# meco-group/omg-tools

Hardware: AMD Instinct MI355X
Metric: MPC solves/sec, 1024-agent Holonomic Point2point batch per GPU (higher is better)
Workload: dtype f64

## Files before the change

### omg-tools_amd/csrc/omgx.hip

```cpp
#include <hip/hip_runtime.h>
#include <hip/hip_ext.h>
#include <stdarg.h>
#include <stdio.h>
#include <stdlib.h>
#include <string.h>
#include <string>
#include <vector>
#include "../../include/omgx.h"
#include "omgx_core.h"
#include "omgx_plan.h"
#include "omgx_kernels.h"
#include "omgx_table_cache.h"

namespace {

thread_local std::string g_err;

#define HIPCHK(call)                                                              \
  do {                                                                            \
    hipError_t e_ = (call);                                                       \
    if (e_ != hipSuccess) {                                                       \
      g_err = std::string(#call) + ": " + hipGetErrorString(e_);                  \
      return OMGX_E_HIP;                                                          \
    }                                                                             \
// ... 343 lines not shown
        if (ad >= 0) { b->ev_hess.push_back(ad); b->ev_hess.push_back(plan.order[q1]); b->ev_hess.push_back(plan.order[q2]); }
      }
  }
  UP(prog, 6 * d.n_prog); UP(knots, t->n_knots); UP(pp_ptr, t->n_pp + 1); UP(pm_coef, t->n_mono);
  UP(pm_ptr, t->n_mono + 1); UP(pm_atom, t->n_matom); UP(slot_pp, d.n_slots);
  if (d.mono_packed == 2) {
    TRY(upload(img, plan.pm_rec8.data(), plan.pm_rec8.size(), (const omgx::MonoRec8**)&b->dev.pm_rec));
    TRY(upload(img, plan.sl_ell8.data(), plan.sl_ell8.size(), (const omgx::MonoRec8**)&b->dev.sl_ell));
  } else { UP(pm_rec, plan.pm_rec.size()); UP(sl_ell, plan.sl_ell.size()); }
  UP(row_ptr, d.n_con + 2); UP(t_coef, d.n_terms); UP(t_slot, d.n_terms); UP(t_var, OMGX_TERM_VARS * d.n_terms);
  UP(order, d.N); UP(leaf_off, d.n_leaf + 1); UP(leaf_bw, plan.leaf_bw.size()); UP(blk, d.N);
  UP(eq_rows, d.n_eq); UP(eq_index, d.n_con);
  UP(cpl_ptr, d.n_leaf + 1); UP(cpl_idx, plan.cpl_idx.size()); UP(cpl_map, plan.cpl_map.size());
  UP(d_off, d.n_leaf + 1); UP(b_off, plan.b_off.size());
  UP(lf_w, plan.lf_w.size()); UP(lf_ldb, plan.lf_ldb.size()); UP(lf_band, plan.lf_band.size()); UP(lf_kind, plan.lf_kind.size()); UP(dl_pos, plan.dl_pos.size());
  UP(pair4, plan.pair4.size()); UP(eqe3, plan.eqe3.size());
  UP(je_row, plan.je_row.size()); UP(diag_addr, d.N); UP(tq_addr, plan.tq_addr.size());
  UP(reg_w, d.N); UP(je_rp, plan.je_rp.size());
  UP(slot_rng, plan.slot_rng.size());
  UP(row_perm, plan.row_perm.size()); UP(cs_ptr, plan.cs_ptr.size()); UP(cs_rec, plan.cs_rec.size());
  UP(obj_ent, plan.obj_ent.size());
  UP(ka_rec, plan.ka_rec.size()); UP(kh_rec, plan.kh_rec.size()); UP(kg_rec, plan.kg_rec.size());
  UP(ka_fix, plan.ka_fix.size()); UP(kg_fix, plan.kg_fix.size()); UP(kh_fix, plan.kh_fix.size());
  UP(rt_ell, plan.rt_ell.size()); UP(rt_glen, plan.rt_glen.size()); UP(jp_ell, plan.jp_ell.size()); UP(jp_glen, plan.jp_glen.size());
  UP(cs_ell, plan.cs_ell.size()); UP(cs_glen, plan.cs_glen.size()); UP(cs_col, plan.cs_col.size()); UP(cs_own, plan.cs_own.size());
  UP(jv_ell, plan.jv_ell.size()); UP(jv_own, plan.jv_own.size()); UP(jv_glen, plan.jv_glen.size());
  UP(ja_ell, plan.ja_ell.size()); UP(ja_own, plan.ja_own.size()); UP(ja_glen, plan.ja_glen.size());
  UP(sl_list, plan.sl_list.size()); UP(sl_glen, plan.sl_glen.size());
  UP(lift_rec, plan.lift_rec.size()); UP(lift_lev, plan.lift_lev.size());
  return bind_tables(b, img);
// ... 432 lines not shown
    hipExtLaunchKernelGGL(b->inst.prepare, dim3(B), dim3(b->threads), (uint32_t)b->prep_lds, b->stream, e0, nullptr, 0u, d, b->dev, b->opts,
                          kp, kx0, klb, kub, shared ? 1 : 0, (const double*)klam, (const int32_t*)kst, B, b->d_prep, b->prep_doubles, (flags & OMGX_ONLY_FAILED) ? 1 : 0);
    HIPCHK(hipGetLastError());
    e0 = nullptr;
  }
  const StoreArgs* k_stp = (b->store.out || b->signals.log) ? &b->d_store->st : nullptr;
  const int k_only_failed = (flags & OMGX_ONLY_FAILED) ? 1 : 0, k_n_alt = b->d_x0_alt ? b->n_alt : 0;
  const CenterArgs* k_ctr = b->center_on ? b->d_center : nullptr;
  double* k_prep = prepared ? b->d_prep : nullptr;
  const StopArgs* k_stop = b->stop_on ? b->d_stop : nullptr;
  const bool lean_launch = !k_stp && !k_only_failed && !k_n_alt && !b->d_attempts && !k_ctr && !k_prep && !k_stop &&
                           !(b->opts.compl_tol > 0.0) && !(b->opts.viol_tol > 0.0) && !b->opts.refine;
  const Instances& in = b->inst;
  b->last_instance = lean_launch && in.lean ? 1 : 0;
  const ipm_kernel_t kern = b->last_instance ? in.lean : (b->opts.refine && in.refine ? in.refine : in.full);
  hipExtLaunchKernelGGL(kern, dim3(b->n_slabs), dim3(b->threads), (uint32_t)b->lds_bytes, b->stream,
                        e0, e1, 0u, d, b->dev,
                        b->opts, b->kkt_doubles, kp, kx0, klb, kub, shared ? 1 : 0, kx, klam, kst, kit, B, b->d_prof,
                        b->d_slabs, b->slab_doubles, b->d_dw, b->d_order, k_stp, k_only_failed,
                        b->d_next, b->d_x0_alt, k_n_alt, b->d_attempts,
                        (unsigned long long*)(b->d_stats ? b->d_stats + 4 * (size_t)(b->stats_launch++ % b->stats_slots) : nullptr),
                        b->stagger, k_ctr, k_prep, b->prep_doubles, k_stop);
  HIPCHK(hipGetLastError());
  if (ranged)
    hipLaunchKernelGGL(range_contract_lam, dim3((B * nu + 255) / 256), dim3(256), 0, b->stream, (const double*)b->d_lam, lam_user_dev, B, nu, ni,
                       (const int32_t*)b->d_range_dup);
  if (!dev) {
    HIPCHK(hipMemcpyAsync(x, b->d_x, (size_t)B * d.n_var * sizeof(double), hipMemcpyDeviceToHost, b->stream));
    HIPCHK(hipMemcpyAsync(lam_g, ranged ? b->d_lam_user : b->d_lam, (size_t)B * nu * sizeof(double), hipMemcpyDeviceToHost, b->stream));
    HIPCHK(hipMemcpyAsync(status, b->d_status, (size_t)B * sizeof(int32_t), hipMemcpyDeviceToHost, b->stream));
    HIPCHK(hipMemcpyAsync(iters, b->d_iters, (size_t)B * sizeof(int32_t), hipMemcpyDeviceToHost, b->stream));
    HIPCHK(hipStreamSynchronize(b->stream));
  }
  return OMGX_OK;
}
// ... 535 lines not shown
  }
  a.iters_log = sp->iters_log; a.status_log = sp->status_log;
  a.plant = b->plant_on ? b->d_plant : nullptr;
  a.script = b->script_on ? b->d_script : nullptr;
  const ipm_rollout_t kern = b->script_on ? (b->plant_on ? b->inst.rollout_plant_script : b->inst.rollout_script)
                                          : (b->plant_on ? b->inst.rollout_plant : b->inst.rollout);
  HIPCHK(hipMemcpyAsync(b->ro_steps.p, steps.data(), sizeof(RolloutStep) * steps.size(), hipMemcpyHostToDevice, b->stream));
  TRY(push_args(b, &b->d_rollout, a));
  TRY(flush_order(b));
  const bool shared = flags & OMGX_BOUNDS_SHARED;
  hipEvent_t e0 = b->ext_ev0, e1 = b->ext_ev0 ? b->ext_ev1 : nullptr;
  b->ext_ev0 = b->ext_ev1 = nullptr;
  b->timed = false;
  hipExtLaunchKernelGGL(kern, dim3(b->n_slabs < b->n_agents ? b->n_slabs : b->n_agents), dim3(b->threads), (uint32_t)b->lds_bytes, b->stream, e0, e1, 0u,
                        d, b->dev, b->opts, b->kkt_doubles, p, x, lbg, ubg, shared ? 1 : 0, lam_g, status, iters, b->n_agents,
                        b->d_slabs, b->slab_doubles, b->d_dw, b->d_next, (const RolloutArgs*)b->d_rollout, b->stagger, b->d_order,
                        (const StoreArgs*)((b->store.out || b->signals.log) ? &b->d_store->st : nullptr));
  HIPCHK(hipGetLastError());
  return OMGX_OK;
}

int omgx_batch_predict_ex(omgx_batch* b, const double* x, double* p, int32_t coeff_off, int32_t n_spl, int32_t degree,
                          const double* knots, int32_t n_knots, double tau, double inv_T, int32_t n_out,
                          const int32_t* p_off, int32_t p_t, double t_value, int32_t mode, const double* state_in,
                          int32_t n_sub, double dtau) {
  const Plan pl{coeff_off, n_spl, degree, n_knots, inv_T, knots};
  TRY(check_predict("predict", pl, 1, kAnySpl, x, p, p_off, n_out));
  if (mode != OMGX_PREDICT_IDEAL && mode != OMGX_PREDICT_RK4) return bad("predict: mode = %d is neither OMGX_PREDICT_IDEAL nor OMGX_PREDICT_RK4", mode);
  if (mode == OMGX_PREDICT_RK4 && (!state_in || n_sub < 1 || !(dtau > 0.0) || n_out < 2))
    return bad("predict: OMGX_PREDICT_RK4 needs state_in, n_sub >= 1, dtau > 0 and n_out >= 2");
  PredictArgs a;
// ... 226 lines not shown
```

### omg-tools_amd/csrc/omgx_core.h

```cpp
#pragma once
#include <stdint.h>
#include <math.h>

#ifdef OMGX_HOST_PORT
#define OMGX_FN inline
#define OMGX_HD inline
#else
#define OMGX_FN __device__ __forceinline__
#define OMGX_HD __host__ __device__ inline
#endif

#ifdef OMGX_HOST_PORT
#include <vector>
static thread_local std::vector<double> omgx_rbak;
#endif
#ifdef OMGX_COUNT_FACT
#include <atomic>
static std::atomic<long> omgx_dbg_nfact(0);
static std::atomic<long> omgx_dbg_cnt[12];
#endif
namespace omgx {

enum { ROW_FREE = 0, ROW_UPPER = 1, ROW_LOWER = 2, ROW_EQ = 3, ROW_BAD = 4 };
enum { OP_DIV = 0, OP_BSPL = 1, OP_COS = 2, OP_SIN = 3 };
// ... 38 lines not shown
struct RowTerm { double coef; int32_t slot; int16_t v0, v1, v2, v3; };
struct HItem { double coef; int32_t row, target; int16_t slot, vthird, vfourth, kind; };

struct Tables {
  const int32_t* prog; const double* knots;
  const int32_t* pp_ptr; const double* pm_coef; const int32_t* pm_ptr; const int32_t* pm_atom;
  const int32_t* slot_pp;
  const MonoRec* pm_rec;
  const int32_t* slot_rng;
  const int32_t* row_ptr; const double* t_coef; const int32_t* t_slot; const int32_t* t_var;
  const int32_t* order; const int32_t* leaf_off; const int32_t* blk;
  const int32_t* eq_rows; const int32_t* eq_index;
  const int32_t* cpl_ptr; const int32_t* cpl_idx; const int32_t* cpl_map;
  const int32_t* d_off; const int32_t* b_off;
  const int32_t* lf_w; const int32_t* lf_ldb; const int32_t* lf_band; const int32_t* lf_kind; const int32_t* dl_pos;
  const int32_t* eqe3;
  const int32_t* pair4;
  const int32_t* je_row; const int32_t* diag_addr;
  const int32_t* je_rp;
  const double* reg_w;
  const int32_t* leaf_bw;
  const int32_t* tq_addr;
  const int32_t* row_perm;
  const RowTerm* rt_ell;
  const int32_t* rt_glen;
  const int32_t* jp_ell;
  const int32_t* jp_glen;
  const int32_t* cs_ell;
  const int32_t* cs_glen;
  const int32_t* cs_own;
// ... 276 lines not shown
  __device__ int nwaves() const { return blockDim.x >> 6; }
  __device__ void wave_sync() const {
    if (kHbm) { __builtin_amdgcn_fence(__ATOMIC_RELEASE, "workgroup"); __builtin_amdgcn_wave_barrier(); __builtin_amdgcn_fence(__ATOMIC_ACQUIRE, "workgroup"); }
    else { __builtin_amdgcn_fence(__ATOMIC_RELEASE, "wavefront"); __builtin_amdgcn_wave_barrier(); __builtin_amdgcn_fence(__ATOMIC_ACQUIRE, "wavefront"); }
  }
};
typedef CtxT<false> Ctx;
#endif

#define OMGX_PFOR(i, n) for (int i = c.tid(); i < (n); i += c.nthr())
#define OMGX_PFOR_U4(i, n) _Pragma("unroll 4") for (int i = c.tid(); i < (n); i += c.nthr())

enum { PH_JAC = 0, PH_RESID, PH_ASSEMBLE, PH_FACTOR, PH_SOLVE, PH_STEP, PH_LINESEARCH, PH_UPDATE, PH_F_LEAF, PH_F_SCHUR, PH_F_ROOT, PH_LA, PH_LS, PH_LB, PH_SETUP, PH_TOTAL,
       PH_S_DESC, PH_S_PARAMS, PH_S_JAC0, PH_S_CLASS, PH_S_INIT, PH_A_ZERO, PH_A_PAIRS, PH_A_REST, PH_A_DIAG,
       PH_K_FWD, PH_K_ROOTRHS, PH_K_ROOT, PH_K_LEAFRHS, PH_K_BWD, PH_L_TERMS, PH_L_ROWS,
       PH_F_PARK, PH_F_SWEEP, PH_F_SCALE, PH_A_TCOL, PH_A_HESS, PH_P_LOAD, PH_P_DIV, PH_P_BSPL, PH_P_SLOTS, PH_COUNT };
#if defined(OMGX_PROFILE) && !defined(OMGX_HOST_PORT)
#define OMGX_TIC() long long tic_ = (c.sync(), clock64())
#define OMGX_TOC(k) do { c.sync(); long long now_ = clock64(); if (c.tid() == 0 && c.prof) c.prof[k] += now_ - tic_; tic_ = now_; } while (0)
#else
#define OMGX_TIC() do {} while (0)
#define OMGX_TOC(k) do {} while (0)
#endif

OMGX_FN double pp_eval(const Tables& T, int pp, const double* a) {
  double tot = 0.0;
  for (int m = T.pp_ptr[pp]; m < T.pp_ptr[pp + 1]; ++m) {
    double v = T.pm_coef[m];
    for (int q = T.pm_ptr[m]; q < T.pm_ptr[m + 1]; ++q) v *= a[T.pm_atom[q]];
    tot += v;
  }
// ... 287 lines not shown
  for (int t = T.row_ptr[r] + c.tid(); t < T.row_ptr[r + 1]; t += c.nthr()) {
    double v = term_coef(T, w, t);
    const int32_t* tv = T.t_var + OMGX_TV * t;
    for (int k = 0; k < OMGX_TV && tv[k] >= 0; ++k) v *= xv[tv[k]];
    g += v;
  }
  return g;
}

OMGX_FN int tri(int i, int k) { return i * (i + 1) / 2 + k; }

struct Kkt {
  const int32_t *d_off, *b_off, *leaf_off, *leaf_bw, *cpl_ptr, *cpl_idx, *blk, *cpl_map, *lf_w, *lf_ldb, *lf_band, *lf_kind, *dl_pos;
  int n_leaf, n_root, root_off;
  double* a;
  OMGX_FN void bind(const Dims& dd, const Tables& TT, double* store) {
    d_off = TT.d_off; b_off = TT.b_off; leaf_off = TT.leaf_off; leaf_bw = TT.leaf_bw; cpl_ptr = TT.cpl_ptr;
    cpl_idx = TT.cpl_idx; blk = TT.blk; cpl_map = TT.cpl_map;
    lf_w = TT.lf_w; lf_ldb = TT.lf_ldb; lf_band = TT.lf_band; lf_kind = TT.lf_kind; dl_pos = TT.dl_pos;
    n_leaf = dd.n_leaf; n_root = dd.n_root; root_off = dd.root_off; a = store;
  }
  OMGX_FN double* P(int l) const { return a + d_off[l]; }
  OMGX_FN int ld(int l) const { return b_off[l]; }
  OMGX_FN double* R() const { return a + d_off[n_leaf]; }
  OMGX_FN int nl(int l) const { return leaf_off[l + 1] - leaf_off[l]; }
  OMGX_FN int nc(int l) const { return cpl_ptr[l + 1] - cpl_ptr[l]; }
};

struct BMat { int a, ld, nfact, rows, npos, dinv, pan, cpl, bw, pad_; };
static_assert(sizeof(BMat) <= OMGX_BMAT_DOUBLES * sizeof(double), "BMat larger than its LDS slot");
#define OMGX_NB 4
#define OMGX_PAN_SMALL(n) (4 * (n) + 16)

#define OMGX_PANEL_STRIDES(C, M, sr, sc) const int sr = C::hbm ? 1 : (M).ld, sc = C::hbm ? (M).ld : 1
OMGX_FN int baddr(const BMat& M, int r, int k) { return M.a + r * M.ld + (M.ld == 0 ? 1 : 0) * ((r * (r + 1)) >> 1) + k; }
template <int KIND>
OMGX_FN int baddr_k(const BMat& M, int r, int k) {
  return KIND == 1 ? M.a + r * M.ld + k : (KIND == 2 ? M.a + ((r * (r + 1)) >> 1) + k : baddr(M, r, k));
}

#ifdef OMGX_HOST_PORT
// ... 339 lines not shown
          const double bv = (kb < M.nfact) ? bv_l * iv_l : 0.0;
          acc = __builtin_amdgcn_mfma_f64_16x16x4f64(av, bv, acc, 0, 0, 0);
#pragma unroll
          for (int i = 0; i < 4; ++i) if (ok[i]) A[ad[i]] = acc[i];
        }
      }
      tile0 += tr;
#endif
    }
    c.sync();
    OMGX_TOC(PH_LB);
  }
  *bad = c.rmax(badl ? 1.0 : 0.0) > 0.0 ? 1 : 0;
}

template <class C>
OMGX_FN void kkt_describe(const C& c, const Dims& d, const Kkt& K, Work& w, bool sync_after = true) {
  const int who = c.nthr() > 64 ? 64 : 0;
  BMat* Ms = (BMat*)w.col;
  double* stage = w.col + OMGX_BMAT_DOUBLES * (OMGX_MAX_LEAF + 1);
  const int pan0 = (int)(stage + OMGX_STAGE_LD * (OMGX_MAX_LEAF + 1) - w.col);
  if (c.tid() == who) {
    int pan = pan0;
    for (int l = 0; l < d.n_leaf; ++l) {
      BMat& M = Ms[l];
      if constexpr (C::wave_only) {
        M.a = K.d_off[l]; M.ld = K.ld(l); M.nfact = K.nl(l); M.rows = K.nl(l) + K.nc(l) + 1; M.npos = M.nfact;
        M.dinv = K.leaf_off[l]; M.pan = K.lf_w[l]; M.cpl = K.cpl_ptr[l]; M.bw = K.lf_kind[l] ? -1 : K.lf_band[l]; M.pad_ = K.lf_ldb[l];
        continue;
      }
      M.a = K.d_off[l]; M.ld = K.ld(l); M.nfact = K.nl(l); M.rows = K.nl(l) + K.nc(l) + 1; M.npos = M.nfact;
      M.dinv = K.leaf_off[l]; M.pan = pan; pan += C::hbm ? OMGX_PAN_SMALL(M.nfact) : OMGX_PAN_LD * M.rows; M.cpl = K.cpl_ptr[l]; M.bw = K.leaf_bw[l];
    }
    BMat& Mr = Ms[d.n_leaf];
    Mr.a = C::root_lds ? 0 : K.d_off[d.n_leaf]; Mr.ld = 0; Mr.nfact = d.nr; Mr.rows = d.nr + 1; Mr.npos = d.n_root; Mr.dinv = -1; Mr.pan = pan0; Mr.cpl = 0; Mr.bw = d.nr;
    Mr.pad_ = K.d_off[d.n_leaf];
  }
  if (sync_after) c.sync();
}

#ifndef OMGX_HOST_PORT
OMGX_FN WPanel wpanel_leaf(const BMat& M) {
  WPanel P; P.base = M.a; P.ld = M.ld; P.n = M.nfact; P.nreg = M.rows - 2; P.nvec = 2; P.npos = M.nfact; P.bw = M.bw;
  P.vrow = M.rows - 2; P.band = M.bw; P.ldb = M.pad_; P.wbase = M.pan;
  return P;
}
OMGX_FN WPanel wpanel_root(const BMat& M, int n_root) {
  WPanel P; P.base = M.a; P.ld = 0; P.n = M.nfact; P.nreg = M.nfact; P.nvec = 1; P.npos = n_root; P.bw = M.nfact;
  P.vrow = M.nfact; P.band = -1; P.ldb = 0; P.wbase = 0;
  return P;
}

struct DiagLeaf { int base, n, S, dinv, dl; };
// ... 760 lines not shown
}

struct Start { int status, warm, use_t; double mu, zt, f; };

template <class C> OMGX_HD double opt_compl_tol(const Opts& o) { if constexpr (C::lean) return 0.0; else return o.compl_tol; }
template <class C> OMGX_HD double opt_viol_tol(const Opts& o) { if constexpr (C::lean) return 0.0; else return o.viol_tol; }

template <class C>
OMGX_FN Start ipm_setup(const C& c, const Dims& d, const Tables& T, const Opts& o, Work& w,
                        const double* p, const double* x0, const double* lb, const double* ub,
                        const double* lam0, int prev_status, int kkt_doubles, bool describe = true) {
  const int n = d.n_var, m = d.n_con;
  Start res; res.status = 1; res.warm = 0; res.use_t = 0; res.mu = o.mu_init; res.zt = 0.0; res.f = 0.0;
  OMGX_TIC();
  if constexpr (!C::prep) {
    if (describe) {
      Kkt K; K.bind(d, T, w.kkt);
      kkt_describe(c, d, K, w, false);
    }
  }

  const bool warm_in = o.warm_start && prev_status == 0;
  const double compl_tol = opt_compl_tol<C>(o);
  const double tol_c = (compl_tol > 0.0 && compl_tol < o.tol) ? compl_tol : o.tol;
  OMGX_PFOR(i, n) w.x[i] = x0[i];
  if constexpr (!C::prep) { if (warm_in) { OMGX_PFOR(r, m) w.ds[r] = lam0[r]; } }
  if (c.tid() == 0) w.x[n] = 1.0;
  eval_params(c, d, T, w, p);
  OMGX_TOC(PH_S_PARAMS);
  if constexpr (C::general) {
    lift_project(c, d, T, w, m, w.x);
    if (d.n_lift > 0) {
      double bad_aux = 0.0;
      OMGX_PFOR(k, d.n_lift) if (!isfinite(w.x[n - d.n_lift + k])) bad_aux = 1.0;
// ... 788 lines not shown
  return res;
}

template <class C>
OMGX_FN Result ipm_solve(const C& c, const Dims& d, const Tables& T, const Opts& o, Work& w,
                         const double* p, const double* x0, const double* lb, const double* ub,
                         const double* lam0, int prev_status, int kkt_doubles, double dw_prev = 0.0) {
  const Start st = ipm_setup(c, d, T, o, w, p, x0, lb, ub, lam0, prev_status, kkt_doubles);
  return ipm_iterate(c, d, T, o, w, lb, ub, st, kkt_doubles, dw_prev);
}

template <class C>
OMGX_FN void ipm_eval(const C& c, const Dims& d, const Tables& T, Work& w, const double* p, const double* x,
                      const double* lam, int kkt_doubles, double* f_out) {
  const int n = d.n_var, m = d.n_con;
  Kkt K; K.bind(d, T, w.kkt);
  kkt_describe(c, d, K, w);
  OMGX_PFOR(i, n) w.x[i] = x[i];
  if (c.tid() == 0) w.x[n] = 0.0;
  eval_params(c, d, T, w, p);
  jac_entries4(c, T.ja_ell, T.ja_own, T.ja_glen, d.n_ja4, w, w.x, [&](int e, int, double v) { w.jval[e] = v; });
  OMGX_PFOR(i, m) { const int r = T.row_perm[i]; w.hv[r] = row_value_ell<C>(d, T, w, i, m, w.x); }
  OMGX_PFOR(r, m) w.ht[r] = lam[r];
  OMGX_PFOR(i, kkt_doubles) w.kkt[i] = 0.0;
  const double f = c.rsum(row_value_share(c, T, w, m, w.x));
  if (c.tid() == 0) *f_out = f;
  c.sync();
  for (int bin = c.tid(); bin < d.n_owner; bin += c.nthr()) hess_bin<C>(d, T, w, m, bin, d.dump_off + (bin & 63));
  c.sync();
  hess_fix(c, d, T, w);
}

// ... 2 lines not shown
```

### omg-tools_amd/csrc/omgx_kernels.h

```cpp
#pragma once

struct KnotArg { double k[40]; };
#define OMGX_SAMPLE_CHUNK 1024

struct CenterArgs {
  int x_spl, p_rel, n_dim, L;
  double* x_i;
  const int32_t* pub_inv;
  double* x_send;
};
struct StopArgs {
  int o_state, o_input, o_pose, n_dim;
  double tol;
  int32_t* under_way;
};
struct StoreArgs {
  double* out;
  double* v_tot;
  const double* t0;
  int coeff_off, n_spl, degree, n_knots, n_der, n_samp;
  double dt, inv_T;
  KnotArg knots;
};
struct SignalArgs {
// ... 152 lines not shown
      double s2 = 0.0;
      for (int k = 0; k < n_spl; ++k) { const double dd = lg[(size_t)k * cap + n - 1] - target[(size_t)b * n_spl + k]; s2 = s2 + dd * dd; }
      dist = sqrt(s2);
      if (n_der >= 2) {
        s2 = 0.0;
        for (int k = 0; k < n_spl; ++k) { const double v = lg[((size_t)n_spl + k) * cap + n - 1]; s2 = s2 + v * v; }
        vlast = sqrt(s2);
      }
    }
    double* sm = summary + (size_t)b * 8;
    sm[0] = (double)n; sm[1] = n >= 1 ? (n - 1) * sample_time : 0.0; sm[2] = path; sm[3] = vmax; sm[4] = amax;
    sm[5] = dist; sm[6] = vlast; sm[7] = 0.0;
  }
}

template <int MODE, bool WAVE_ONLY, bool GEN, bool REFINE = false, bool LEAN = false>
__global__ void __launch_bounds__(512)
ipm_solve_kernel(omgx::Dims d, omgx::Tables T, omgx::Opts o, int kkt_doubles,
                 const double* __restrict__ p, const double* __restrict__ x0,
                 const double* __restrict__ lb, const double* __restrict__ ub, int bounds_shared,
                 double* __restrict__ x, double* __restrict__ lam, int32_t* __restrict__ status,
                 int32_t* __restrict__ iters, int n_agents, long long* __restrict__ prof,
                 double* __restrict__ slabs, size_t slab_doubles, double* __restrict__ dw_state,
                 const int32_t* __restrict__ order, const StoreArgs* __restrict__ stp, int only_failed,
                 int* __restrict__ next_slot, const double* __restrict__ x0_alt, int n_alt, int32_t* __restrict__ attempts,
                 unsigned long long* __restrict__ stats, int stagger, const CenterArgs* __restrict__ ctr,
                 double* __restrict__ prep, size_t prep_doubles, const StopArgs* __restrict__ stop) {
  extern __shared__ __align__(16) double lds[];
  omgx::Work w;
    omgx::work_carve_split<MODE>(w, lds, MODE == omgx::WS_LDS ? nullptr : slabs + (size_t)blockIdx.x * slab_doubles,
                               d, kkt_doubles);
  omgx::CtxT<omgx::ws_kkt_hbm(MODE), WAVE_ONLY, omgx::ws_root_lds(MODE), GEN, false, REFINE, LEAN> c; c.red = w.red;
#ifdef OMGX_PROFILE
  __shared__ long long prof_lds[omgx::PH_COUNT];
  c.prof = prof_lds;
#else
  c.prof = nullptr;
#endif
  [[maybe_unused]] double* const jval_own = w.jval;
  const bool describe_once = LEAN || prep != nullptr || stp == nullptr;
  if (describe_once) { omgx::Kkt K0; K0.bind(d, T, w.kkt); omgx::kkt_describe(c, d, K0, w, true); }
  __shared__ int slot_lds;
  if (stagger > 0 && (__builtin_amdgcn_s_getreg(6148) & 1))
    for (int i = 0; i < stagger; ++i) __builtin_amdgcn_s_sleep(127);
  for (int slot = blockIdx.x; slot < n_agents;) {
    const int b = order ? order[slot] : slot;
    if (!next_slot) slot += gridDim.x;
    else {
      if (threadIdx.x == 0) slot_lds = gridDim.x + atomicAdd(next_slot, 1);
      __syncthreads();
      slot = slot_lds;
      __syncthreads();
    }
    if constexpr (!LEAN) { if (only_failed && status[b] == 0) continue; }
    if constexpr (!LEAN)
    if (stop) {
      const StopArgs sa = *stop;
      bool go = sa.under_way[b] != 0;
      if (go && omgx::stop_criterium(p + (size_t)b * d.n_par, sa.o_state, sa.o_input, sa.o_pose, sa.n_dim, sa.tol)) go = false;
      if (!go) {
        for (int i = threadIdx.x; i < d.n_var; i += blockDim.x) x[(size_t)b * d.n_var + i] = x0[(size_t)b * d.n_var + i];
        if (threadIdx.x == 0) { sa.under_way[b] = 0; iters[b] = 0; }
        continue;
      }
    }
#ifdef OMGX_PROFILE
    if (threadIdx.x < omgx::PH_COUNT) prof_lds[threadIdx.x] = 0;
    __syncthreads();
    const long long t_begin = clock64();
#endif
    const double* lbb = lb + (bounds_shared ? 0 : (size_t)b * d.n_con);
    const double* ubb = ub + (bounds_shared ? 0 : (size_t)b * d.n_con);
    omgx::Result r;
    int attempt = 0;
    if constexpr (LEAN) {
      const omgx::Start st = omgx::ipm_setup(c, d, T, o, w, p + (size_t)b * d.n_par, x0 + (size_t)b * d.n_var, lbb, ubb,
                                             o.warm_start ? lam + (size_t)b * d.n_con : nullptr, o.warm_start ? status[b] : 0, kkt_doubles, false);
      r = omgx::ipm_iterate(c, d, T, o, w, lbb, ubb, st, kkt_doubles, o.warm_start ? dw_state[b] : 0.0);
      __builtin_amdgcn_s_setprio(0);
      __syncthreads();
    } else
    for (;;) {
      const double* xs = attempt == 0 ? x0 + (size_t)b * d.n_var : x0_alt + ((size_t)(attempt - 1) * n_agents + b) * d.n_var;
      omgx::Start st;
// ... 36 lines not shown
        ca.x_i[(size_t)b * ns + q] = v;
        if (slot >= 0) ca.x_send[(size_t)slot * ns + q] = v;
      }
    }
    if constexpr (!LEAN)
    if (stp) {
      const StoreArgs st = *stp;
      if (st.out) {
        __syncthreads();
        sample_agent<double>(w.x + st.coeff_off, w.kkt, st.n_spl, st.degree, st.knots, st.n_knots, st.n_der, st.t0[b],
                             st.dt, st.inv_T, st.n_samp, 0, st.n_samp, st.out + (size_t)b * st.n_der * st.n_spl * st.n_samp,
                             st.v_tot ? st.v_tot + (size_t)b * st.n_samp : nullptr);
      }
      const SignalArgs& sg = reinterpret_cast<const StoreBlock*>(stp)->sg;
      if (sg.log) signals_append_agent(sg, b, w.x + sg.coeff_off, p[(size_t)b * d.n_par + sg.p_t], w.kkt);
      if (prep) { __syncthreads(); omgx::Kkt K0; K0.bind(d, T, w.kkt); omgx::kkt_describe(c, d, K0, w, true); }
    }
#ifdef OMGX_PROFILE
    __syncthreads();
    if (threadIdx.x == 0) prof_lds[omgx::PH_TOTAL] = clock64() - t_begin;
    __syncthreads();
    if (prof && threadIdx.x < omgx::PH_COUNT) prof[(size_t)b * omgx::PH_COUNT + threadIdx.x] = prof_lds[threadIdx.x];
#endif
    __syncthreads();
  }
  if (next_slot && threadIdx.x == 0) {
    __threadfence();
    if (atomicAdd(next_slot + 1, 1) == (int)gridDim.x - 1) { next_slot[0] = 0; next_slot[1] = 0; __threadfence(); }
  }
}

__host__ __device__ inline size_t prepare_lds_doubles(const omgx::Dims& d) {
  return (size_t)d.n_slots + d.n_atoms + d.n_knots + d.N + 64;
}
template <bool GEN>
__global__ void __launch_bounds__(512, 4)
ipm_prepare_kernel(omgx::Dims d, omgx::Tables T, omgx::Opts o, const double* __restrict__ p, const double* __restrict__ x0,
                   const double* __restrict__ lb, const double* __restrict__ ub, int bounds_shared,
                   const double* __restrict__ lam, const int32_t* __restrict__ status, int n_agents,
                   double* __restrict__ prep, size_t prep_doubles, int only_failed) {
  extern __shared__ __align__(16) double lds[];
  const int b = blockIdx.x;
  if (b >= n_agents) return;
  if (only_failed && status[b] == 0) return;
// ... 632 lines not shown
};

template <int MODE, bool WAVE_ONLY, bool GEN, bool PLANT = false, bool SCRIPT = false>
__global__ void __launch_bounds__(512)
ipm_rollout_kernel(omgx::Dims d, omgx::Tables T, omgx::Opts o, int kkt_doubles, double* __restrict__ p, double* __restrict__ x,
                   const double* __restrict__ lb, const double* __restrict__ ub, int bounds_shared, double* __restrict__ lam,
                   int32_t* __restrict__ status, int32_t* __restrict__ iters, int n_agents, double* __restrict__ slabs,
                   size_t slab_doubles, double* __restrict__ dw_state, int* __restrict__ next_slot,
                   const RolloutArgs* __restrict__ rop, int stagger, const int32_t* __restrict__ order,
                   const StoreArgs* __restrict__ stp) {
  extern __shared__ __align__(16) double lds[];
  omgx::Work w;
  omgx::work_carve_split<MODE>(w, lds, MODE == omgx::WS_LDS ? nullptr : slabs + (size_t)blockIdx.x * slab_doubles, d, kkt_doubles);
  omgx::CtxT<omgx::ws_kkt_hbm(MODE), WAVE_ONLY, omgx::ws_root_lds(MODE), GEN> c; c.red = w.red;
  c.prof = nullptr;
  __shared__ int slot_lds;
  if (stagger > 0 && (__builtin_amdgcn_s_getreg(6148) & 1))
    for (int i = 0; i < stagger; ++i) __builtin_amdgcn_s_sleep(127);
  const int K = rop->K;
  for (int slot = blockIdx.x; slot < n_agents;) {
    const int b = order ? order[slot] : slot;
    if (threadIdx.x == 0) slot_lds = gridDim.x + atomicAdd(next_slot, 1);
    __syncthreads();
    slot = slot_lds;
    __syncthreads();
    double* pb = p + (size_t)b * d.n_par;
    double* xb = x + (size_t)b * d.n_var;
    double* lamb = lam + (size_t)b * d.n_con;
    const double* lbb = lb + (bounds_shared ? 0 : (size_t)b * d.n_con);
    const double* ubb = ub + (bounds_shared ? 0 : (size_t)b * d.n_con);
    for (int k = 0; k < K; ++k) {
      const RolloutStep st = rop->steps[k];
      if constexpr (PLANT) {
        if (!plant_predict_agent(rop->plant->pl, b, xb + rop->plant->pl.coeff_off, pb, st.tau, st.t_rel, w.kkt)) {
          if (threadIdx.x == 0) {
            iters[b] = 0;
            for (int k2 = k; k2 < K; ++k2) {
              if (rop->iters_log) rop->iters_log[(size_t)k2 * n_agents + b] = 0;
              if (rop->status_log) rop->status_log[(size_t)k2 * n_agents + b] = status[b];
            }
// ... 81 lines not shown
          sample_agent<double>(w.x + st2.coeff_off, w.kkt, st2.n_spl, st2.degree, st2.knots, st2.n_knots, st2.n_der, st2.t0[b],
                               st2.dt, st2.inv_T, st2.n_samp, 0, st2.n_samp, st2.out + (size_t)b * st2.n_der * st2.n_spl * st2.n_samp,
                               st2.v_tot ? st2.v_tot + (size_t)b * st2.n_samp : nullptr);
        }
        if constexpr (!PLANT) {
        const SignalArgs& sg = reinterpret_cast<const StoreBlock*>(stp)->sg;
        if (sg.log) signals_append_agent(sg, b, w.x + sg.coeff_off, pb[sg.p_t], w.kkt);
        }
      }
      if constexpr (PLANT) {
        const PlantBlock* pk = rop->plant;
        plant_simulate_agent(pk->pl, pk->sg.log ? &pk->sg : nullptr, b, w.x + pk->pl.coeff_off, pb[pk->pl.p_t], w.kkt);
      }
      __syncthreads();
    }
  }
  if (threadIdx.x == 0) {
    __threadfence();
    if (atomicAdd(next_slot + 1, 1) == (int)gridDim.x - 1) { next_slot[0] = 0; next_slot[1] = 0; }
  }
}

__global__ void admm_center_kernel(omgx_admm_layout lay, const double* __restrict__ x, int n_var,
                                   const double* __restrict__ p, int n_par, double* __restrict__ x_i, int B,
                                   const int32_t* __restrict__ pub_rows, int n_pub, double* __restrict__ x_send) {
  const int ns = lay.n_dim * lay.L;
  const int i = blockIdx.x * blockDim.x + threadIdx.x;
  if (i >= (B + n_pub) * ns) return;
  const int row = i / ns, q = i - row * ns, k = q / lay.L;
  const int b = row < B ? row : pub_rows[row - B];
  const double v = x[(size_t)b * n_var + lay.x_spl + q] + p[(size_t)b * n_par + lay.p_rel + k];
  if (row < B) x_i[i] = v; else x_send[(size_t)(row - B) * ns + q] = v;
}

__global__ void __launch_bounds__(256)
// ... 180 lines not shown
```

### omg-tools_amd/csrc/omgx_plan.h

```cpp
#pragma once
#include <stdlib.h>
#include <algorithm>
#include <array>
#include <cmath>
#include <map>
#include <functional>
#include <numeric>
#include <queue>
#include <set>
#include <string>
#include <vector>
#include "../../include/omgx.h"
#include "omgx_core.h"

namespace omgx {

struct HostPlan {
  Dims dims;
  Tables tables;
  int kkt_doubles;
  std::vector<int32_t> order, pos, blk, leaf_off, leaf_bw, eq_rows, eq_index;
  std::vector<int32_t> jr_ptr, jr_pos, t_jidx, row_leaf, cpl_ptr, cpl_idx, cpl_map;
  std::vector<int32_t> d_off, b_off;
  std::vector<int32_t> lf_w, lf_ldb, lf_band, lf_kind, dl_pos;
  std::vector<std::vector<std::vector<int>>> var_cpl;
  std::vector<int32_t> pair4, eqe3, je_row, jt_addr, diag_addr, t_row, tq_addr;
  std::vector<double> reg_w;
  std::vector<MonoRec> pm_rec;
  std::vector<MonoRec8> pm_rec8, sl_ell8;
  std::vector<int32_t> je_rp, slot_rng;
  struct HessTerm { double coef; int32_t slot, row; int nv; int32_t v[OMGX_TV], p[OMGX_TV], ha[OMGX_TV * (OMGX_TV - 1) / 2]; };
  std::vector<HessTerm> hrec;
  std::vector<int32_t> je_ptr, jv_list, row_perm, cs_ptr, cs_rec, obj_ent;
  std::vector<JItem> je_item;
  std::vector<int32_t> ka_rec, ka_fix, kg_fix, kh_fix;
  std::vector<RowTerm> rt_ell;
  std::vector<JItem> jv_ell, ja_ell;
  std::vector<MonoRec> sl_ell;
  std::vector<int32_t> ja_own, jv_own, ja_glen, sl_list, sl_glen;
// ... 729 lines not shown
        }
      }
      d.n_kafix = (int)ka_fix.size() / 3; d.n_kgfix = (int)kg_fix.size() / 3; d.n_khfix = (int)kh_fix.size() / 3;
      if (kh_fix.empty()) kh_fix.assign(3, 0);
      if (ka_fix.empty()) ka_fix.assign(3, 0);
      if (kg_fix.empty()) kg_fix.assign(3, 0);
      d.side_off = side0;
      d.n_owner = owners;
      kkt_doubles = side0 + n_side + 64;
      d.dump_off = side0 + n_side;
      T.ka_rec = ka_rec.data(); T.kh_rec = kh_rec.data(); T.kg_rec = kg_rec.data();
      T.ka_fix = ka_fix.data(); T.kg_fix = kg_fix.data(); T.kh_fix = kh_fix.data();
    }
    if (pair4.empty()) pair4.assign(4, 0);
    T.pair4 = pair4.data();
    return true;
  }
};

}
```

Measured before the change: 3.324 million.

## Precompute KKT block descriptors on host and pipeline the work-queue slot fetch

Adds a host-built image of the per-leaf BMat descriptors in compact (wave-only) mode, which the kernel copies cooperatively instead of having one thread compute them serially. The dynamic agent queue now fetches the next slot at the start of each agent's solve into a double-buffered LDS slot, which drops two barriers per agent. The queue is skipped entirely when the slab count covers all agents. Queue reset now uses relaxed atomic exchanges instead of threadfences. Profiling also gains head and tail idle-time phases.

```diff
diff --git a/omg-tools_amd/csrc/omgx.hip b/omg-tools_amd/csrc/omgx.hip
--- a/omg-tools_amd/csrc/omgx.hip
+++ b/omg-tools_amd/csrc/omgx.hip
@@ -381,6 +381,7 @@
   UP(cpl_ptr, d.n_leaf + 1); UP(cpl_idx, plan.cpl_idx.size()); UP(cpl_map, plan.cpl_map.size());
   UP(d_off, d.n_leaf + 1); UP(b_off, plan.b_off.size());
   UP(lf_w, plan.lf_w.size()); UP(lf_ldb, plan.lf_ldb.size()); UP(lf_band, plan.lf_band.size()); UP(lf_kind, plan.lf_kind.size()); UP(dl_pos, plan.dl_pos.size());
+  UP(bmat_img, plan.bmat_img.size());
   UP(pair4, plan.pair4.size()); UP(eqe3, plan.eqe3.size());
   UP(je_row, plan.je_row.size()); UP(diag_addr, d.N); UP(tq_addr, plan.tq_addr.size());
   UP(reg_w, d.N); UP(je_rp, plan.je_rp.size());
@@ -843,11 +844,12 @@
   const Instances& in = b->inst;
   b->last_instance = lean_launch && in.lean ? 1 : 0;
   const ipm_kernel_t kern = b->last_instance ? in.lean : (b->opts.refine && in.refine ? in.refine : in.full);
+  int* const k_next = b->n_slabs >= B ? nullptr : b->d_next;
   hipExtLaunchKernelGGL(kern, dim3(b->n_slabs), dim3(b->threads), (uint32_t)b->lds_bytes, b->stream,
                         e0, e1, 0u, d, b->dev,
                         b->opts, b->kkt_doubles, kp, kx0, klb, kub, shared ? 1 : 0, kx, klam, kst, kit, B, b->d_prof,
                         b->d_slabs, b->slab_doubles, b->d_dw, b->d_order, k_stp, k_only_failed,
-                        b->d_next, b->d_x0_alt, k_n_alt, b->d_attempts,
+                        k_next, b->d_x0_alt, k_n_alt, b->d_attempts,
                         (unsigned long long*)(b->d_stats ? b->d_stats + 4 * (size_t)(b->stats_launch++ % b->stats_slots) : nullptr),
                         b->stagger, k_ctr, k_prep, b->prep_doubles, k_stop);
   HIPCHK(hipGetLastError());
@@ -1413,7 +1415,7 @@
   b->timed = false;
   hipExtLaunchKernelGGL(kern, dim3(b->n_slabs < b->n_agents ? b->n_slabs : b->n_agents), dim3(b->threads), (uint32_t)b->lds_bytes, b->stream, e0, e1, 0u,
                         d, b->dev, b->opts, b->kkt_doubles, p, x, lbg, ubg, shared ? 1 : 0, lam_g, status, iters, b->n_agents,
-                        b->d_slabs, b->slab_doubles, b->d_dw, b->d_next, (const RolloutArgs*)b->d_rollout, b->stagger, b->d_order,
+                        b->d_slabs, b->slab_doubles, b->d_dw, b->n_slabs >= b->n_agents ? nullptr : b->d_next, (const RolloutArgs*)b->d_rollout, b->stagger, b->d_order,
                         (const StoreArgs*)((b->store.out || b->signals.log) ? &b->d_store->st : nullptr));
   HIPCHK(hipGetLastError());
   return OMGX_OK;
diff --git a/omg-tools_amd/csrc/omgx_core.h b/omg-tools_amd/csrc/omgx_core.h
--- a/omg-tools_amd/csrc/omgx_core.h
+++ b/omg-tools_amd/csrc/omgx_core.h
@@ -5,9 +5,11 @@
 #ifdef OMGX_HOST_PORT
 #define OMGX_FN inline
 #define OMGX_HD inline
+#define OMGX_HDF inline
 #else
 #define OMGX_FN __device__ __forceinline__
 #define OMGX_HD __host__ __device__ inline
+#define OMGX_HDF __host__ __device__ __forceinline__
 #endif
 
 #ifdef OMGX_HOST_PORT
@@ -76,6 +78,7 @@
   const int32_t* cpl_ptr; const int32_t* cpl_idx; const int32_t* cpl_map;
   const int32_t* d_off; const int32_t* b_off;
   const int32_t* lf_w; const int32_t* lf_ldb; const int32_t* lf_band; const int32_t* lf_kind; const int32_t* dl_pos;
+  const int32_t* bmat_img;
   const int32_t* eqe3;
   const int32_t* pair4;
   const int32_t* je_row; const int32_t* diag_addr;
@@ -382,7 +385,9 @@
 enum { PH_JAC = 0, PH_RESID, PH_ASSEMBLE, PH_FACTOR, PH_SOLVE, PH_STEP, PH_LINESEARCH, PH_UPDATE, PH_F_LEAF, PH_F_SCHUR, PH_F_ROOT, PH_LA, PH_LS, PH_LB, PH_SETUP, PH_TOTAL,
        PH_S_DESC, PH_S_PARAMS, PH_S_JAC0, PH_S_CLASS, PH_S_INIT, PH_A_ZERO, PH_A_PAIRS, PH_A_REST, PH_A_DIAG,
        PH_K_FWD, PH_K_ROOTRHS, PH_K_ROOT, PH_K_LEAFRHS, PH_K_BWD, PH_L_TERMS, PH_L_ROWS,
-       PH_F_PARK, PH_F_SWEEP, PH_F_SCALE, PH_A_TCOL, PH_A_HESS, PH_P_LOAD, PH_P_DIV, PH_P_BSPL, PH_P_SLOTS, PH_COUNT };
+       PH_F_PARK, PH_F_SWEEP, PH_F_SCALE, PH_A_TCOL, PH_A_HESS, PH_P_LOAD, PH_P_DIV, PH_P_BSPL, PH_P_SLOTS,
+       PH_WG_HEAD, PH_WG_TAIL,
+       PH_COUNT };
 #if defined(OMGX_PROFILE) && !defined(OMGX_HOST_PORT)
 #define OMGX_TIC() long long tic_ = (c.sync(), clock64())
 #define OMGX_TOC(k) do { c.sync(); long long now_ = clock64(); if (c.tid() == 0 && c.prof) c.prof[k] += now_ - tic_; tic_ = now_; } while (0)
@@ -700,17 +705,17 @@
   const int32_t *d_off, *b_off, *leaf_off, *leaf_bw, *cpl_ptr, *cpl_idx, *blk, *cpl_map, *lf_w, *lf_ldb, *lf_band, *lf_kind, *dl_pos;
   int n_leaf, n_root, root_off;
   double* a;
-  OMGX_FN void bind(const Dims& dd, const Tables& TT, double* store) {
+  OMGX_HDF void bind(const Dims& dd, const Tables& TT, double* store) {
     d_off = TT.d_off; b_off = TT.b_off; leaf_off = TT.leaf_off; leaf_bw = TT.leaf_bw; cpl_ptr = TT.cpl_ptr;
     cpl_idx = TT.cpl_idx; blk = TT.blk; cpl_map = TT.cpl_map;
     lf_w = TT.lf_w; lf_ldb = TT.lf_ldb; lf_band = TT.lf_band; lf_kind = TT.lf_kind; dl_pos = TT.dl_pos;
     n_leaf = dd.n_leaf; n_root = dd.n_root; root_off = dd.root_off; a = store;
   }
   OMGX_FN double* P(int l) const { return a + d_off[l]; }
-  OMGX_FN int ld(int l) const { return b_off[l]; }
+  OMGX_HDF int ld(int l) const { return b_off[l]; }
   OMGX_FN double* R() const { return a + d_off[n_leaf]; }
-  OMGX_FN int nl(int l) const { return leaf_off[l + 1] - leaf_off[l]; }
-  OMGX_FN int nc(int l) const { return cpl_ptr[l + 1] - cpl_ptr[l]; }
+  OMGX_HDF int nl(int l) const { return leaf_off[l + 1] - leaf_off[l]; }
+  OMGX_HDF int nc(int l) const { return cpl_ptr[l + 1] - cpl_ptr[l]; }
 };
 
 struct BMat { int a, ld, nfact, rows, npos, dinv, pan, cpl, bw, pad_; };
@@ -1080,29 +1085,44 @@
   *bad = c.rmax(badl ? 1.0 : 0.0) > 0.0 ? 1 : 0;
 }
 
+template <bool WAVE_ONLY, bool HBM, bool ROOT_LDS>
+OMGX_HDF void kkt_describe_fill(const Dims& d, const Kkt& K, BMat* Ms) {
+  const int pan0 = (OMGX_BMAT_DOUBLES + OMGX_STAGE_LD) * (OMGX_MAX_LEAF + 1);
+  int pan = pan0;
+  for (int l = 0; l < d.n_leaf; ++l) {
+    BMat& M = Ms[l];
+    if constexpr (WAVE_ONLY) {
+      M.a = K.d_off[l]; M.ld = K.ld(l); M.nfact = K.nl(l); M.rows = K.nl(l) + K.nc(l) + 1; M.npos = M.nfact;
+      M.dinv = K.leaf_off[l]; M.pan = K.lf_w[l]; M.cpl = K.cpl_ptr[l]; M.bw = K.lf_kind[l] ? -1 : K.lf_band[l]; M.pad_ = K.lf_ldb[l];
+      continue;
+    }
+    M.a = K.d_off[l]; M.ld = K.ld(l); M.nfact = K.nl(l); M.rows = K.nl(l) + K.nc(l) + 1; M.npos = M.nfact;
+    M.dinv = K.leaf_off[l]; M.pan = pan; pan += HBM ? OMGX_PAN_SMALL(M.nfact) : OMGX_PAN_LD * M.rows; M.cpl = K.cpl_ptr[l]; M.bw = K.leaf_bw[l];
+  }
+  BMat& Mr = Ms[d.n_leaf];
+  Mr.a = ROOT_LDS ? 0 : K.d_off[d.n_leaf]; Mr.ld = 0; Mr.nfact = d.nr; Mr.rows = d.nr + 1; Mr.npos = d.n_root; Mr.dinv = -1; Mr.pan = pan0; Mr.cpl = 0; Mr.bw = d.nr;
+  Mr.pad_ = K.d_off[d.n_leaf];
+}
+
 template <class C>
 OMGX_FN void kkt_describe(const C& c, const Dims& d, const Kkt& K, Work& w, bool sync_after = true) {
   const int who = c.nthr() > 64 ? 64 : 0;
-  BMat* Ms = (BMat*)w.col;
-  double* stage = w.col + OMGX_BMAT_DOUBLES * (OMGX_MAX_LEAF + 1);
-  const int pan0 = (int)(stage + OMGX_STAGE_LD * (OMGX_MAX_LEAF + 1) - w.col);
-  if (c.tid() == who) {
-    int pan = pan0;
-    for (int l = 0; l < d.n_leaf; ++l) {
-      BMat& M = Ms[l];
-      if constexpr (C::wave_only) {
-        M.a = K.d_off[l]; M.ld = K.ld(l); M.nfact = K.nl(l); M.rows = K.nl(l) + K.nc(l) + 1; M.npos = M.nfact;
-        M.dinv = K.leaf_off[l]; M.pan = K.lf_w[l]; M.cpl = K.cpl_ptr[l]; M.bw = K.lf_kind[l] ? -1 : K.lf_band[l]; M.pad_ = K.lf_ldb[l];
-        continue;
-      }
-      M.a = K.d_off[l]; M.ld = K.ld(l); M.nfact = K.nl(l); M.rows = K.nl(l) + K.nc(l) + 1; M.npos = M.nfact;
-      M.dinv = K.leaf_off[l]; M.pan = pan; pan += C::hbm ? OMGX_PAN_SMALL(M.nfact) : OMGX_PAN_LD * M.rows; M.cpl = K.cpl_ptr[l]; M.bw = K.leaf_bw[l];
-    }
-    BMat& Mr = Ms[d.n_leaf];
-    Mr.a = C::root_lds ? 0 : K.d_off[d.n_leaf]; Mr.ld = 0; Mr.nfact = d.nr; Mr.rows = d.nr + 1; Mr.npos = d.n_root; Mr.dinv = -1; Mr.pan = pan0; Mr.cpl = 0; Mr.bw = d.nr;
-    Mr.pad_ = K.d_off[d.n_leaf];
-  }
+  if (c.tid() == who) kkt_describe_fill<C::wave_only, C::hbm, C::root_lds>(d, K, (BMat*)w.col);
   if (sync_after) c.sync();
+}
+
+template <class C>
+OMGX_FN void kkt_descriptors(const C& c, const Dims& d, const Tables& T, Work& w, bool sync_after = true) {
+  if constexpr (C::wave_only) {
+    const int t0 = c.nthr() > 64 ? 64 : 0, nt = c.nthr() > 64 ? 64 : c.nthr();
+    const int i0 = c.tid() - t0, n = (d.n_leaf + 1) * (int)(sizeof(BMat) / sizeof(int32_t));
+    int32_t* Ms = (int32_t*)w.col;
+    if (i0 >= 0 && i0 < nt) for (int i = i0; i < n; i += nt) Ms[i] = T.bmat_img[i];
+    if (sync_after) c.sync();
+  } else {
+    Kkt K; K.bind(d, T, w.kkt);
+    kkt_describe(c, d, K, w, sync_after);
+  }
 }
 
 #ifndef OMGX_HOST_PORT
@@ -1893,10 +1913,7 @@
   Start res; res.status = 1; res.warm = 0; res.use_t = 0; res.mu = o.mu_init; res.zt = 0.0; res.f = 0.0;
   OMGX_TIC();
   if constexpr (!C::prep) {
-    if (describe) {
-      Kkt K; K.bind(d, T, w.kkt);
-      kkt_describe(c, d, K, w, false);
-    }
+    if (describe) kkt_descriptors(c, d, T, w, false);
   }
 
   const bool warm_in = o.warm_start && prev_status == 0;
@@ -2715,8 +2732,7 @@
 OMGX_FN void ipm_eval(const C& c, const Dims& d, const Tables& T, Work& w, const double* p, const double* x,
                       const double* lam, int kkt_doubles, double* f_out) {
   const int n = d.n_var, m = d.n_con;
-  Kkt K; K.bind(d, T, w.kkt);
-  kkt_describe(c, d, K, w);
+  kkt_descriptors(c, d, T, w);
   OMGX_PFOR(i, n) w.x[i] = x[i];
   if (c.tid() == 0) w.x[n] = 0.0;
   eval_params(c, d, T, w, p);
diff --git a/omg-tools_amd/csrc/omgx_kernels.h b/omg-tools_amd/csrc/omgx_kernels.h
--- a/omg-tools_amd/csrc/omgx_kernels.h
+++ b/omg-tools_amd/csrc/omgx_kernels.h
@@ -190,6 +190,13 @@
   }
 }
 
+__device__ __forceinline__ void queue_leave(int* next_slot) {
+  if (atomicAdd(next_slot + 1, 1) == (int)gridDim.x - 1) {
+    __hip_atomic_exchange(next_slot, 0, __ATOMIC_RELAXED, __HIP_MEMORY_SCOPE_AGENT);
+    __hip_atomic_exchange(next_slot + 1, 0, __ATOMIC_RELAXED, __HIP_MEMORY_SCOPE_AGENT);
+  }
+}
+
 template <int MODE, bool WAVE_ONLY, bool GEN, bool REFINE = false, bool LEAN = false>
 __global__ void __launch_bounds__(512)
 ipm_solve_kernel(omgx::Dims d, omgx::Tables T, omgx::Opts o, int kkt_doubles,
@@ -202,6 +209,10 @@
                  int* __restrict__ next_slot, const double* __restrict__ x0_alt, int n_alt, int32_t* __restrict__ attempts,
                  unsigned long long* __restrict__ stats, int stagger, const CenterArgs* __restrict__ ctr,
                  double* __restrict__ prep, size_t prep_doubles, const StopArgs* __restrict__ stop) {
+#ifdef OMGX_PROFILE
+  long long t_mark = clock64();
+  int b_last = -1;
+#endif
   extern __shared__ __align__(16) double lds[];
   omgx::Work w;
     omgx::work_carve_split<MODE>(w, lds, MODE == omgx::WS_LDS ? nullptr : slabs + (size_t)blockIdx.x * slab_doubles,
@@ -215,20 +226,16 @@
 #endif
   [[maybe_unused]] double* const jval_own = w.jval;
   const bool describe_once = LEAN || prep != nullptr || stp == nullptr;
-  if (describe_once) { omgx::Kkt K0; K0.bind(d, T, w.kkt); omgx::kkt_describe(c, d, K0, w, true); }
-  __shared__ int slot_lds;
+  if (describe_once) omgx::kkt_descriptors(c, d, T, w, true);
+  __shared__ int slot_lds[2];
+  int slot_par = 0;
   if (stagger > 0 && (__builtin_amdgcn_s_getreg(6148) & 1))
     for (int i = 0; i < stagger; ++i) __builtin_amdgcn_s_sleep(127);
   for (int slot = blockIdx.x; slot < n_agents;) {
     const int b = order ? order[slot] : slot;
-    if (!next_slot) slot += gridDim.x;
-    else {
-      if (threadIdx.x == 0) slot_lds = gridDim.x + atomicAdd(next_slot, 1);
-      __syncthreads();
-      slot = slot_lds;
-      __syncthreads();
-    }
-    if constexpr (!LEAN) { if (only_failed && status[b] == 0) continue; }
+    if (next_slot && threadIdx.x == 0) slot_lds[slot_par] = gridDim.x + atomicAdd(next_slot, 1);
+    const auto next_agent = [&]() { slot = next_slot ? slot_lds[slot_par] : slot + (int)gridDim.x; slot_par ^= 1; };
+    if constexpr (!LEAN) { if (only_failed && status[b] == 0) { __syncthreads(); next_agent(); continue; } }
     if constexpr (!LEAN)
     if (stop) {
       const StopArgs sa = *stop;
@@ -237,6 +244,8 @@
       if (!go) {
         for (int i = threadIdx.x; i < d.n_var; i += blockDim.x) x[(size_t)b * d.n_var + i] = x0[(size_t)b * d.n_var + i];
         if (threadIdx.x == 0) { sa.under_way[b] = 0; iters[b] = 0; }
+        __syncthreads();
+        next_agent();
         continue;
       }
     }
@@ -244,6 +253,8 @@
     if (threadIdx.x < omgx::PH_COUNT) prof_lds[threadIdx.x] = 0;
     __syncthreads();
     const long long t_begin = clock64();
+    if (threadIdx.x == 0) prof_lds[omgx::PH_WG_HEAD] = t_begin - t_mark;
+    b_last = b;
 #endif
     const double* lbb = lb + (bounds_shared ? 0 : (size_t)b * d.n_con);
     const double* ubb = ub + (bounds_shared ? 0 : (size_t)b * d.n_con);
@@ -310,20 +321,24 @@
       }
       const SignalArgs& sg = reinterpret_cast<const StoreBlock*>(stp)->sg;
       if (sg.log) signals_append_agent(sg, b, w.x + sg.coeff_off, p[(size_t)b * d.n_par + sg.p_t], w.kkt);
-      if (prep) { __syncthreads(); omgx::Kkt K0; K0.bind(d, T, w.kkt); omgx::kkt_describe(c, d, K0, w, true); }
+      if (prep) { __syncthreads(); omgx::kkt_descriptors(c, d, T, w, true); }
     }
 #ifdef OMGX_PROFILE
     __syncthreads();
     if (threadIdx.x == 0) prof_lds[omgx::PH_TOTAL] = clock64() - t_begin;
     __syncthreads();
     if (prof && threadIdx.x < omgx::PH_COUNT) prof[(size_t)b * omgx::PH_COUNT + threadIdx.x] = prof_lds[threadIdx.x];
+    t_mark = clock64();
 #endif
     __syncthreads();
-  }
-  if (next_slot && threadIdx.x == 0) {
-    __threadfence();
-    if (atomicAdd(next_slot + 1, 1) == (int)gridDim.x - 1) { next_slot[0] = 0; next_slot[1] = 0; __threadfence(); }
-  }
+    next_agent();
+  }
+  if (next_slot && threadIdx.x == 0) queue_leave(next_slot);
+#ifdef OMGX_PROFILE
+  if (threadIdx.x == 0) prof_lds[omgx::PH_WG_TAIL] = clock64() - t_mark;
+  __syncthreads();
+  if (prof && b_last >= 0 && threadIdx.x == omgx::PH_WG_TAIL) prof[(size_t)b_last * omgx::PH_COUNT + omgx::PH_WG_TAIL] = prof_lds[omgx::PH_WG_TAIL];
+#endif
 }
 
 __host__ __device__ inline size_t prepare_lds_doubles(const omgx::Dims& d) {
@@ -986,16 +1001,14 @@
   omgx::work_carve_split<MODE>(w, lds, MODE == omgx::WS_LDS ? nullptr : slabs + (size_t)blockIdx.x * slab_doubles, d, kkt_doubles);
   omgx::CtxT<omgx::ws_kkt_hbm(MODE), WAVE_ONLY, omgx::ws_root_lds(MODE), GEN> c; c.red = w.red;
   c.prof = nullptr;
-  __shared__ int slot_lds;
+  __shared__ int slot_lds[2];
+  int slot_par = 0;
   if (stagger > 0 && (__builtin_amdgcn_s_getreg(6148) & 1))
     for (int i = 0; i < stagger; ++i) __builtin_amdgcn_s_sleep(127);
   const int K = rop->K;
   for (int slot = blockIdx.x; slot < n_agents;) {
     const int b = order ? order[slot] : slot;
-    if (threadIdx.x == 0) slot_lds = gridDim.x + atomicAdd(next_slot, 1);
-    __syncthreads();
-    slot = slot_lds;
-    __syncthreads();
+    if (next_slot && threadIdx.x == 0) slot_lds[slot_par] = gridDim.x + atomicAdd(next_slot, 1);
     double* pb = p + (size_t)b * d.n_par;
     double* xb = x + (size_t)b * d.n_var;
     double* lamb = lam + (size_t)b * d.n_con;
@@ -1107,11 +1120,11 @@
       }
       __syncthreads();
     }
-  }
-  if (threadIdx.x == 0) {
-    __threadfence();
-    if (atomicAdd(next_slot + 1, 1) == (int)gridDim.x - 1) { next_slot[0] = 0; next_slot[1] = 0; }
-  }
+    __syncthreads();
+    slot = next_slot ? slot_lds[slot_par] : slot + (int)gridDim.x;
+    slot_par ^= 1;
+  }
+  if (next_slot && threadIdx.x == 0) queue_leave(next_slot);
 }
 
 __global__ void admm_center_kernel(omgx_admm_layout lay, const double* __restrict__ x, int n_var,
diff --git a/omg-tools_amd/csrc/omgx_plan.h b/omg-tools_amd/csrc/omgx_plan.h
--- a/omg-tools_amd/csrc/omgx_plan.h
+++ b/omg-tools_amd/csrc/omgx_plan.h
@@ -23,6 +23,7 @@
   std::vector<int32_t> jr_ptr, jr_pos, t_jidx, row_leaf, cpl_ptr, cpl_idx, cpl_map;
   std::vector<int32_t> d_off, b_off;
   std::vector<int32_t> lf_w, lf_ldb, lf_band, lf_kind, dl_pos;
+  std::vector<int32_t> bmat_img;
   std::vector<std::vector<std::vector<int>>> var_cpl;
   std::vector<int32_t> pair4, eqe3, je_row, jt_addr, diag_addr, t_row, tq_addr;
   std::vector<double> reg_w;
@@ -782,6 +783,12 @@
     }
     if (pair4.empty()) pair4.assign(4, 0);
     T.pair4 = pair4.data();
+    bmat_img.assign(compact ? (size_t)(d.n_leaf + 1) * (sizeof(BMat) / sizeof(int32_t)) : 1, 0);
+    if (compact) {
+      Kkt K; K.bind(d, T, nullptr);
+      kkt_describe_fill<true, false, false>(d, K, (BMat*)bmat_img.data());
+    }
+    T.bmat_img = bmat_img.data();
     return true;
   }
 };
```

Measured after the change: 3.545 million (median of 6 runs). 6.7% higher.
